# martinResearch/PySparseLP

Hardware: AMD Instinct MI355X
Metric: admm_iterations_per_sec (higher is better)
Workload: dtype f64

## Files before the change

### pysparselp_amd/csrc/slp_tall.h

```cpp
#pragma once
#include "slp_common.h"
#include "slp_tall_item.h"

namespace slp {

constexpr int kTallC = 4096;
constexpr int kTallT = 1024;
constexpr int kTallSlots = 8;
constexpr int kTallDepth = 4;
constexpr int kTallBuckets = 6;
constexpr int kTallCellShift = kTallIdBits + kTallColBits + kTallRowBits;
static_assert(kTallBuckets * 32 == 3 * kWave, "k_tall_build scans the (count, bank class) buckets three per lane of one wave");
static_assert(1 + kTallDictMax + kTallRmax <= (1 << kTallRowBits), "an item's sum field: scratch cell, value table, the block's rows (slp_tall_item.h)");
static_assert(kTallRmax + 1 < (1 << kTallRowBits) && kTallC == (1 << kTallColBits) && kTallDictMax == (1 << kTallIdBits), "tall geometry");
static_assert(kTallT == kTallPlanLanes && kTallC == kTallCmax, "the planner's constants (slp_tall_plan.h)");
static_assert((kTallRmaxSplit + 1) * 8 + kTallDictMax * 8 + 2 * kTallC * 8 <= kTallLdsBytes, "tall cells: LDS budget");

constexpr unsigned int kPktNewCell = 0x80000000u;
constexpr unsigned int kNoTile = 0x7fffffffu;
constexpr unsigned int kOob = 0xffffff00u;

struct TallPkt {
    unsigned int off;
    unsigned int xsrc;
    unsigned int c[4];
    unsigned int strip;
    unsigned int pad;
};
static_assert(sizeof(TallPkt) == 32, "packet header");

__host__ __device__ inline unsigned long long tall_value_key(unsigned long long bits) {
    return (bits >> 63) ? ~bits : (bits | 0x8000000000000000ull);
}

}
```

### pysparselp_amd/csrc/slp_tall.hip

```cpp
#include <atomic>
#include <cmath>
#include <cstdlib>
#include <cstring>
#include <vector>

#include <rocprim/rocprim.hpp>

#include "slp_common.h"
#include "slp_kernels.h"
#include "slp_tall.h"

namespace slp {


__global__ void k_tall_range(i64 nrow, const i64 *__restrict__ ptr, const i32 *__restrict__ idx, i64 c0, i64 c1,
                             i64 *__restrict__ lo, i64 *__restrict__ len) {
    for (i64 r = (i64)blockIdx.x * blockDim.x + threadIdx.x; r < nrow; r += (i64)gridDim.x * blockDim.x) {
        const i64 s = ptr[r], e = ptr[r + 1];
        auto lower = [&](i64 c) {
            i64 a = s, b = e;
            while (a < b) {
                const i64 mid = (a + b) >> 1;
                if ((i64)idx[mid] < c) a = mid + 1;
                else b = mid;
// ... 473 lines not shown
                        tall_scan_put(sc, cell, 2ull, bw + cell_w, bp + cell_p);
                        sc.before_w[cell] = bw;
                        sc.before_p[cell] = bp;
                        s_before_w = bw;
                        s_before_p = bp;
                    }
                }
                __syncthreads();
                SLP_TB_PROF(9);
                if (s_cell < ncell && p * 16 < s_n) {
                    const unsigned int *g = reinterpret_cast<const unsigned int *>(keys + s_c0) + p * 32;
                    const unsigned int lds = __builtin_amdgcn_readfirstlane((unsigned int)(size_t)s_dump);
                    unsigned int m0_saved;
                    asm volatile("s_mov_b32 %0, m0\n\ts_mov_b32 m0, %1\n\ts_nop 0\n\tglobal_load_lds_dword %2, off\n\ts_mov_b32 m0, %0"
                                 : "=&s"(m0_saved) : "s"(lds), "v"(g) : "memory");
                }
                fits = (i64)(s_before_w + cell_w) <= cap_w && (i64)(s_before_p + cell_p) <= cap_p;
                pay = spay + s_before_w;
                payv = DICT ? nullptr : spayv + s_before_w;
                pk = sdir + s_before_p;
            }
            if (!fits) break;
            {
                unsigned int *base = pay + woff;
                unsigned int hb0 = 0, hb1 = 0;
#pragma unroll
                for (int j = 0; j < kTallSlots; ++j) {
                    if ((unsigned)p < wd[REC && j < 4 ? 0 : j]) {
                        unsigned int item = 0u, hib = 0u;
                        if (have >> j & 1u) {
                            const unsigned int r1 = ((unsigned int)(key[j] >> (kTallIdBits + kTallColBits)) & ((1u << kTallRowBits) - 1)) + sum0;
                            const unsigned int cl = (unsigned int)(key[j] >> kTallIdBits) & (kTallC - 1);
                            if (DICT) {
                                const TallItem it = tall_item_encode((unsigned int)key[j] & ((1u << kTallIdBits) - 1), cl, r1);
                                item = it.word;
                                hib = it.fifth;
                            } else {
                                item = tall_item64_encode(cl, r1);
                            }
                        }
                        const unsigned int at = tall_packet_item_word(lay, REC, (unsigned)p, j);
                        base[at] = item;
                        if (!DICT) payv[woff + at] = value[j];
                        if (j < 4) hb0 |= hib << (8 * j);
                        else hb1 |= hib << (8 * (j - 4));
                    }
                }
                if (DICT && (unsigned)p < wd[0]) base[lay.fifth0 + p] = hb0;
                if (DICT && (unsigned)p < wd[4]) base[lay.fifth1 + p] = hb1;
                if (p == 0) {
                    TallPkt h;
                    h.off = woff;
                    h.xsrc = (g == 0) ? (kPktNewCell | tile_of(tn)) : kNoTile;
                    for (int i = 0; i < 4; ++i) h.c[i] = wd[2 * i] | (wd[2 * i + 1] << 16);
                    h.strip = (unsigned int)t;
                    h.pad = 0;
                    pk[npk] = h;
                }
            }
            woff += words;
            ++npk;
            __syncthreads();
            SLP_TB_PROF(10);
        }
    }
}

template <bool DICT>
__global__ __launch_bounds__(kBlock) void k_tall_estimate(i64 ncell, const i64 *__restrict__ cellptr, int records, unsigned long long *__restrict__ est) {
    unsigned long long w = 0, k = 0;
    for (i64 c = (i64)blockIdx.x * kBlock + threadIdx.x; c < ncell; c += (i64)gridDim.x * kBlock) {
        const unsigned long long n = (unsigned long long)(cellptr[c + 1] - cellptr[c]);
        if (!n) continue;
        const unsigned long long L = n < (unsigned)kTallT ? n : (unsigned)kTallT, tau = (n + kTallT - 1) / kTallT;
        const unsigned long long cw = records ? tall_packet_balanced_words(n, kTallT, DICT, true)
                                              : n + L * (tall_packet_lane_words((unsigned int)tau, DICT, false) - tau);
        w += (cw + 3ull) & ~3ull;
        k += (tau + kTallSlots - 1) / kTallSlots;
    }
#pragma unroll
    for (int off = kWave / 2; off; off >>= 1) { w += __shfl_xor(w, off, kWave); k += __shfl_xor(k, off, kWave); }
    if ((threadIdx.x & (kWave - 1)) == 0) { atomicAdd(&est[0], w); atomicAdd(&est[1], k); }
}

__global__ void k_tall_streams(i64 V, i64 T, int S, const i64 *__restrict__ cellptr, TallScan sc, i64 *__restrict__ ext) {
    for (i64 v = (i64)blockIdx.x * blockDim.x + threadIdx.x; v < V; v += (i64)gridDim.x * blockDim.x) {
        const i64 b = v / S, cs = b * T + T * (v % S) / S, ce = b * T + T * (v % S + 1) / S;
        auto before = [&](i64 c, i64 *w, i64 *k) {
            for (--c; c >= 0 && cellptr[c + 1] == cellptr[c];) --c;
            *w = c >= 0 ? (i64)(sc.w[c] & kScanMask) : 0;
            *k = c >= 0 ? (i64)(sc.p[c] & kScanMask) : 0;
        };
        i64 w0, p0, w1, p1;
        before(cs, &w0, &p0);
        before(ce, &w1, &p1);
        ext[4 * v] = w0;
        ext[4 * v + 1] = w1 - w0;
        ext[4 * v + 2] = p0;
        ext[4 * v + 3] = p1 - p0;
    }
}

__global__ void k_tall_dir(i64 ncell, i64 V, i64 T, int S, int C, const i64 *__restrict__ cellptr, TallScan sc, const i64 *__restrict__ ext,
                           const i64 *__restrict__ pkt_ptr, const TallPkt *__restrict__ sdir, TallPkt *__restrict__ dir) {
    const i64 i0 = (i64)blockIdx.x * blockDim.x + threadIdx.x, step = (i64)gridDim.x * blockDim.x;
    for (i64 c = i0; c < ncell; c += step) {
        if (cellptr[c + 1] == cellptr[c]) continue;
        const i64 pk0 = (i64)sc.before_p[c], np = (i64)(sc.p[c] & kScanMask) - pk0, w0 = (i64)sc.before_w[c];
        const i64 b = c / T, t = c % T, v = b * S + (S > 1 ? tall_range_of(t, T, S) : 0);
        TallPkt *out = dir + pkt_ptr[v] + 1 + (pk0 - ext[4 * v + 2]);
        for (i64 j = 0; j < np; ++j) {
            TallPkt h = sdir[pk0 + j];
            h.off += (unsigned int)(w0 - ext[4 * v]);
            out[j] = h;
        }
    }
    for (i64 v = i0; v < V; v += step) {
        const i64 b = v / S, t_begin = T * (v % S) / S, t_end = T * (v % S + 1) / S;
        i64 first = -1;
        for (i64 u = t_begin; u < t_end; ++u)
            if (cellptr[b * T + u + 1] > cellptr[b * T + u]) { first = u; break; }
        TallPkt h;
        h.off = 0; h.xsrc = first >= 0 ? (unsigned int)(first * C) : kNoTile;
        h.c[0] = h.c[1] = h.c[2] = h.c[3] = 0; h.strip = 0; h.pad = 0;
        dir[pkt_ptr[v]] = h;
        h.off = (unsigned int)ext[4 * v + 1];
        h.xsrc = kNoTile;
        for (i64 k = pkt_ptr[v] + 1 + ext[4 * v + 3]; k < pkt_ptr[v + 1]; ++k) dir[k] = h;
    }
}
static int tall_env(const char *name) {
    const char *e = getenv(name);
    return e ? atoi(e) : 0;
}

static i64 tall_pass_nnz() {
    const char *e = getenv("SLP_TALL_PASS_NNZ");
    const i64 v = e ? atoll(e) : 500000000ll;
    return v > 0 ? v : 500000000ll;
}

bool tall_build(const CsrDev &a, bool transposed, StripJds &f, const ValueDict *dict, i64 block_multiple, i64 rows_before, i64 rows_total,
                const TallCarry *carry) {
    Phase ph(transposed ? "tall_build (A^T from the CSR of A)" : "tall_build");
    hipStream_t st = ctx().stream;
    f = StripJds();
    if ((dict && (dict->D <= 0 || dict->D > kTallDictMax)) || a.nrow == 0 || a.ncol == 0 || a.nnz == 0) return false;
    const i64 nrowF = transposed ? a.ncol : a.nrow, ncolF = transposed ? a.nrow : a.ncol;
    if (ncolF * 8 >= ((i64)1 << 31)) return false;
    TallPlanIn pin;
    pin.nrow = nrowF; pin.ncol = ncolF; pin.nnz = a.nnz; pin.D = dict ? dict->D : 0; pin.cus = ctx().num_cu;
    if (!transposed) { pin.block_multiple = block_multiple; pin.rows_before = rows_before; pin.rows_total = rows_total; }
    pin.env_R = std::max(0, tall_env("SLP_TALL_R")); pin.env_C = tall_env("SLP_TALL_C"); pin.env_split = tall_env("SLP_TALL_SPLIT");
    if (const char *e = getenv("SLP_TALL_RECORDS")) pin.env_records = atoi(e) != 0 ? 1 : 0;
    if (carry && carry->C > 0) {
        pin.carry_records = carry->records;
        pin.carry_C = carry->C; pin.carry_dcap = carry->dcap; pin.carry_total = transposed ? 0 : carry->total;
        pin.carry_R = transposed ? carry->R : 0;
        pin.carry_blocks = transposed ? 0 : carry->blocks;
    }
    const TallPlan plan = tall_plan(pin);
    SLP_REQUIRE(plan.lds_bytes <= kTallLdsBytes && plan.build_lds_bytes <= kTallLdsBytes && plan.R >= 1 && plan.R <= kTallRmax,
                "tall_build: the planned geometry does not fit the LDS");
    const int R = plan.R, S = plan.S, Cw = plan.C;
    const bool records = plan.records;
    const i64 T = plan.T;
    const unsigned int sum0 = tall_item_sum_base(plan.dcap);
    SLP_REQUIRE(sum0 + (unsigned int)R <= (1u << kTallRowBits), "tall_build: sum field");
    const i64 B = (nrowF + R - 1) / R, ncell = B * T, V = B * S;
    unsigned int cellbits = 1;
    while (((i64)1 << cellbits) < ncell) ++cellbits;
    if (kTallCellShift + cellbits > 64) return false;
    i64 P = (a.nnz + tall_pass_nnz() - 1) / tall_pass_nnz();
    P = std::max<i64>(1, std::min<i64>(P, B));
    DevBuf<int> bad(1);
    bad.zero();
    if (transposed) {
        hipLaunchKernelGGL(k_tall_sorted, dim3(grid_for(a.nrow * kWave, kBlock)), dim3(kBlock), 0, st, a.nnz, a.idx.p, a.nrow, a.ptr.p, bad.p);
        SLP_HIP(hipGetLastError());
        int hbad = 0;
        bad.download(&hbad, 1);
        if (hbad) return false;
    }
    DevBuf<unsigned long long> sorted((size_t)a.nnz);
    DevBuf<double> svals;
    if (!dict) svals.alloc((size_t)a.nnz);
    {
        Phase p1("  tall: keys + sort");
        DevBuf<i64> lo, len, opos;
        if (transposed) { lo.alloc((size_t)a.nrow); len.alloc((size_t)a.nrow + 1); opos.alloc((size_t)a.nrow + 1); }
        const int D = dict ? dict->D : 0;
        const unsigned long long *dk = dict ? dict->keys.p : (const unsigned long long *)nullptr;
        const unsigned b0 = transposed ? (unsigned)(kTallIdBits + kTallColBits) : (unsigned)kTallCellShift, b1 = (unsigned)kTallCellShift + cellbits;
        i64 done = 0;
        for (i64 pass = 0; pass < P; ++pass) {
            const i64 bb0 = B * pass / P, bb1 = B * (pass + 1) / P;
            if (bb1 == bb0) continue;
            const i64 f0 = bb0 * (i64)R, f1 = std::min<i64>(bb1 * (i64)R, nrowF);
            i64 n_p = 0, obase = 0;
            if (!transposed) {
                i64 ends[2];
                SLP_HIP(hipMemcpyAsync(&ends[0], a.ptr.p + f0, sizeof(i64), hipMemcpyDeviceToHost, st));
                SLP_HIP(hipMemcpyAsync(&ends[1], a.ptr.p + f1, sizeof(i64), hipMemcpyDeviceToHost, st));
                SLP_HIP(hipStreamSynchronize(st));
                obase = ends[0];
                n_p = ends[1] - ends[0];
            } else {
                hipLaunchKernelGGL(k_tall_range, dim3(grid_for(a.nrow, kBlock)), dim3(kBlock), 0, st, a.nrow, a.ptr.p, a.idx.p, f0, f1, lo.p, len.p);
                SLP_HIP(hipGetLastError());
                size_t bytes = 0;
                SLP_HIP(rocprim::exclusive_scan(nullptr, bytes, len.p, opos.p, (i64)0, (size_t)a.nrow + 1, rocprim::plus<i64>(), st));
                DevBuf<char> tmp(bytes);
                SLP_HIP(rocprim::exclusive_scan(tmp.p, bytes, len.p, opos.p, (i64)0, (size_t)a.nrow + 1, rocprim::plus<i64>(), st));
                SLP_HIP(hipMemcpyAsync(&n_p, opos.p + a.nrow, sizeof(i64), hipMemcpyDeviceToHost, st));
                SLP_HIP(hipStreamSynchronize(st));
            }
            if (n_p == 0) continue;
            DevBuf<unsigned long long> keys((size_t)n_p);
            DevBuf<double> kvals;
            if (!dict && transposed) kvals.alloc((size_t)n_p);
            const i64 scan_rows = transposed ? a.nrow : f1 - f0, r0 = transposed ? 0 : f0;
            if (transposed)
                hipLaunchKernelGGL((k_tall_keys<true>), dim3(grid_for(scan_rows * kWave, kBlock)), dim3(kBlock), 0, st, r0, scan_rows, R, T, Cw, (i64)0, D, dk,
                                   a.ptr.p, a.idx.p, a.val.p, lo.p, opos.p, obase, keys.p, kvals.p, bad.p);
            else
                hipLaunchKernelGGL((k_tall_keys<false>), dim3(grid_for(scan_rows * kWave, kBlock)), dim3(kBlock), 0, st, r0, scan_rows, R, T, Cw, (i64)0, D, dk,
                                   a.ptr.p, a.idx.p, a.val.p, (const i64 *)nullptr, (const i64 *)nullptr, obase, keys.p, (double *)nullptr, bad.p);
            SLP_HIP(hipGetLastError());
            size_t bytes = 0;
            if (dict) {
                SLP_HIP(rocprim::radix_sort_keys(nullptr, bytes, keys.p, sorted.p + done, (size_t)n_p, b0, b1, st));
                DevBuf<char> tmp(bytes);
                SLP_HIP(rocprim::radix_sort_keys(tmp.p, bytes, keys.p, sorted.p + done, (size_t)n_p, b0, b1, st));
                SLP_HIP(hipStreamSynchronize(st));
            } else {
                const double *vin = transposed ? kvals.p : a.val.p + obase;
                SLP_HIP(rocprim::radix_sort_pairs(nullptr, bytes, keys.p, sorted.p + done, vin, svals.p + done, (size_t)n_p, b0, b1, st));
                DevBuf<char> tmp(bytes);
                SLP_HIP(rocprim::radix_sort_pairs(tmp.p, bytes, keys.p, sorted.p + done, vin, svals.p + done, (size_t)n_p, b0, b1, st));
                SLP_HIP(hipStreamSynchronize(st));
            }
            done += n_p;
        }
        int hbad = 0;
        bad.download(&hbad, 1);
        if (hbad || done != a.nnz) return false;
    }
    DevBuf<i64> cellptr((size_t)ncell + 1);
    hipLaunchKernelGGL(k_tall_cellptr, dim3(grid_for(a.nnz, kBlock)), dim3(kBlock), 0, st, a.nnz, ncell, sorted.p, cellptr.p);
    SLP_HIP(hipGetLastError());
    Phase p2("  tall: packets (one pass)");
    DevBuf<unsigned long long> scan(4 * (size_t)ncell + 1), est(2);
    TallScan sc;
    sc.w = scan.p; sc.p = scan.p + ncell; sc.ticket = scan.p + 2 * ncell; sc.before_w = sc.ticket + 1; sc.before_p = sc.before_w + ncell;
    est.zero();
    if (dict) hipLaunchKernelGGL((k_tall_estimate<true>), dim3(grid_for(ncell, kBlock)), dim3(kBlock), 0, st, ncell, cellptr.p, records ? 1 : 0, est.p);
    else hipLaunchKernelGGL((k_tall_estimate<false>), dim3(grid_for(ncell, kBlock)), dim3(kBlock), 0, st, ncell, cellptr.p, records ? 1 : 0, est.p);
    SLP_HIP(hipGetLastError());
    unsigned long long hest[2];
    est.download(hest, 2);
    static std::atomic<double> last_needs[2][2][2];
    std::atomic<double> &last_need_slot = last_needs[transposed ? 1 : 0][dict ? 1 : 0][records ? 1 : 0];
    const double last_need = last_need_slot.load();
    const double room = (last_need > 0.5 && last_need < 2.0) ? last_need * 1.003 : 1.10;
    i64 cap_w = (i64)((double)hest[0] * room) + 65536, cap_p = 2 * (i64)hest[1] + 4096;
    if (const char *e = getenv("SLP_TALL_BUILD_ROOM")) cap_w = std::max<i64>(4, (i64)((double)hest[0] * atof(e)));
    i64 tot_w = 0, tot_p = 0;
    DevBuf<i64> ext(4 * (size_t)V);
    std::vector<i64> hext(4 * (size_t)V);
    DevBuf<unsigned int> spay, sdir;
    DevBuf<double> spayv;
    for (int attempt = 0;; ++attempt) {
        spay.release();
        spayv.release();
        spay.alloc((size_t)cap_w + 64);
        sdir.alloc((size_t)cap_p * 8);
        if (!dict) spayv.alloc((size_t)cap_w + 64);
        SLP_HIP(hipMemsetAsync(scan.p, 0, (2 * (size_t)ncell + 1) * sizeof(unsigned long long), st));
        const unsigned grid = (unsigned)std::min<i64>(ncell, (i64)ctx().num_cu);
        auto build = [&](auto kernel) {
            hipLaunchKernelGGL(kernel, dim3(grid), dim3(kTallT), 0, st, R, T, S, Cw, sum0, ncell, sorted.p, dict ? (const double *)nullptr : svals.p, cellptr.p, sc,
                               cap_w, cap_p, reinterpret_cast<TallPkt *>(sdir.p), spay.p, dict ? (double *)nullptr : spayv.p);
        };
        if (dict) { if (records) build(k_tall_build<true, true>); else build(k_tall_build<true, false>); }
        else { if (records) build(k_tall_build<false, true>); else build(k_tall_build<false, false>); }
        hipLaunchKernelGGL(k_tall_streams, dim3(grid_for(V, kBlock)), dim3(kBlock), 0, st, V, T, S, cellptr.p, sc, ext.p);
        SLP_HIP(hipGetLastError());
        ext.download(hext.data(), hext.size());
        tot_w = hext[4 * (V - 1)] + hext[4 * (V - 1) + 1];
        tot_p = hext[4 * (V - 1) + 2] + hext[4 * (V - 1) + 3];
        if (tot_w <= cap_w && tot_p <= cap_p) break;
        SLP_REQUIRE(attempt == 0, "tall_build: the pass with the exact sizes did not fit");
        cap_w = tot_w; cap_p = tot_p;
    }
    sorted.release();
    svals.release();
    std::vector<i64> hbase((size_t)V + 1), hpkt((size_t)V + 1);
    const i64 limit = dict ? ((i64)1 << 28) : ((i64)1 << 27);
    hpkt[0] = 0;
    for (i64 v = 0; v < V; ++v) {
        if (hext[4 * v + 1] >= limit) return false;
        hbase[v] = hext[4 * v];
        const i64 np = 1 + hext[4 * v + 3];
        hpkt[v + 1] = hpkt[v] + (np + 2 * kTallDepth - 1) / (2 * kTallDepth) * (2 * kTallDepth) + 2 * kTallDepth;
    }
    hbase[V] = tot_w;
    DevBuf<i64> dpkt;
    dpkt.upload(hpkt.data(), hpkt.size());
    if (hest[0]) last_need_slot.store((double)tot_w / (double)hest[0]);
    if (cap_w > tot_w + tot_w / 100 + 65536) {
        DevBuf<unsigned int> exact((size_t)tot_w + 64);
        SLP_HIP(hipMemcpyAsync(exact.p, spay.p, (size_t)tot_w * sizeof(unsigned int), hipMemcpyDeviceToDevice, st));
        DevBuf<double> exactv;
        if (!dict) {
            exactv.alloc((size_t)tot_w + 64);
            SLP_HIP(hipMemcpyAsync(exactv.p, spayv.p, (size_t)tot_w * sizeof(double), hipMemcpyDeviceToDevice, st));
        }
        SLP_HIP(hipStreamSynchronize(st));
        spay = std::move(exact);
        spayv = std::move(exactv);
    }
    f.tall_dir.emplace_back((size_t)hpkt[V] * 8);
    f.tall_pay.emplace_back(std::move(spay));
    DevBuf<unsigned int> &dir = f.tall_dir.back(), &pay = f.tall_pay.back();
    double *vals = nullptr;
    if (!dict) { f.tall_val.emplace_back(std::move(spayv)); vals = f.tall_val.back().p; }
    hipLaunchKernelGGL(k_tall_dir, dim3(grid_for(std::max<i64>(ncell, V), kBlock)), dim3(kBlock), 0, st, ncell, V, T, S, Cw, cellptr.p, sc, ext.p, dpkt.p,
                       reinterpret_cast<const TallPkt *>(sdir.p), reinterpret_cast<TallPkt *>(dir.p));
    SLP_HIP(hipGetLastError());
    std::vector<TallWg> wg((size_t)V);
    for (i64 v = 0; v < V; ++v) {
        const i64 b = v / S;
        wg[(size_t)v].dir = dir.p + hpkt[v] * 8;
        wg[(size_t)v].pay = pay.p + hbase[v];
        wg[(size_t)v].val = vals ? vals + hbase[v] : nullptr;
        wg[(size_t)v].dict = nullptr;
        wg[(size_t)v].npk = hpkt[v + 1] - hpkt[v];
        wg[(size_t)v].row0 = (v % S) * nrowF + b * (i64)R;
        wg[(size_t)v].x0 = 0;
        wg[(size_t)v].ncol = ncolF;
        wg[(size_t)v].nrows = (int)std::min<i64>(R, nrowF - b * (i64)R);
        wg[(size_t)v].D = dict ? dict->D : 0;
    }
    if (S > 1 && V > 8) {
        const i64 q = V / 8, r = V % 8;
        std::vector<TallWg> placed((size_t)V);
        for (i64 orig = 0; orig < V; ++orig) {
            const i64 xcd = orig % 8;
            const i64 pos = (xcd < r ? xcd * (q + 1) : r * (q + 1) + (xcd - r) * q) + orig / 8;
            const i64 sr = pos / B, b = pos % B;
            placed[(size_t)orig] = wg[(size_t)(b * S + sr)];
        }
        wg.swap(placed);
    }
    f.tall_wg.upload(wg.data(), wg.size());
    SLP_HIP(hipStreamSynchronize(st));
    f.tall_bytes = (dir.n + (size_t)tot_w) * sizeof(unsigned int) + (vals ? (size_t)tot_w * sizeof(double) : 0) + wg.size() * sizeof(TallWg) +
                   (dict ? (size_t)dict->D * sizeof(double) : 0);
    f.nrow = nrowF; f.ncol = ncolF; f.nnz = a.nnz; f.T = T; f.B = B; f.C = (int)Cw; f.rpl = 1;
    f.D = dict ? dict->D : 0;
    f.dict = dict ? dict->values.p : nullptr;
    f.tall = true;
    f.tall_R = R;
    f.tall_dcap = plan.dcap;
    f.tall_records = records;
    f.tall_total = plan.total;
    f.S = S;
    if (S > 1) f.part.alloc((size_t)S * (size_t)nrowF);
    f.ok = true;
    return true;
}

bool tall_wanted(i64 nrow, i64 ncol, i64 nnz) {
    const char *e = getenv("SLP_TALL");
    if (e && e[0] == '0') return false;
    const char *m = getenv("SLP_STRIP_MIN_NNZ");
    const i64 min_nnz = m ? atoll(m) : 30000000ll;
    if (nnz < min_nnz || nrow <= 0 || ncol <= 0) return false;
    const double per_cell = ((double)nnz / (double)nrow) / (double)((ncol + kTallC - 1) / kTallC);
    return per_cell >= 0.05 && per_cell < 2.5;
}

}
```

### pysparselp_amd/csrc/slp_tall_spmv.hip

```cpp
#include <cmath>
#include <cstdlib>
#include <cstring>
#include <type_traits>
#include <vector>

#include "slp_common.h"
#include "slp_kernels.h"
#include "slp_tall.h"

namespace slp {


template <bool DICT>
struct TallRegs {
    unsigned int lo[kTallSlots];
    unsigned int hi[DICT ? 2 : 1];
    double val[DICT ? 1 : kTallSlots];
    double x[4];
};

template <bool DICT, bool ACC, bool POW = false, int CT = 0, bool REC = false>
__global__ __launch_bounds__(kTallT) void k_tall_spmv(int nseg, const TallWg *__restrict__ wgs, const double *__restrict__ dict_arg,
                                                      const double *__restrict__ x, double *__restrict__ out, double pw, const int cw,
                                                      const int dcap, const int oxt) {
    const int C = CT ? CT : cw;
    constexpr int kDepth = DICT ? kTallDepth : 2;
    extern __shared__ __attribute__((aligned(16))) double tall_lds[];
    double *const dv = tall_lds + kTallItemTableByte / 8;
    double *const acc = tall_lds + tall_item_sum_base(dcap);
    double *const xt = tall_lds + oxt;
    typedef __attribute__((address_space(3))) double lds_double;
    auto lds_at = [](unsigned int a) -> lds_double & { return *(lds_double *)(unsigned long long)a; };
    const unsigned int lds0 = (unsigned int)(unsigned long long)(lds_double *)tall_lds;
    if (lds0 != 0u) __builtin_trap();
    const unsigned int xtb = 8u * (unsigned int)oxt;
    const int p = threadIdx.x;
    const unsigned int wbase = (unsigned int)__builtin_amdgcn_readfirstlane(p & ~(kWave - 1));
    const bool piece0 = (int)wbase < (C >> 1), piece1 = (int)wbase + kTallT < (C >> 1);
    const int v = blockIdx.x;
    int cur = 0;
    TallWg wg = wgs[v];
    if (p == 0) tall_lds[0] = 0.0;
    for (int r = p; r < wg.nrows; r += kTallT) acc[r] = ACC ? out[wg.row0 + r] : 0.0;
  for (int seg = 0; seg < nseg; ++seg) {
    if (seg > 0) wg = wgs[(i64)seg * gridDim.x + v];
    if (DICT) {
        const double *__restrict__ dsrc = dict_arg ? dict_arg : wg.dict;
        for (int q = p; q < wg.D; q += kTallT) dv[q] = dsrc[q];
    }
    typedef const unsigned int __attribute__((address_space(1))) *gptr_t;
    const gptr_t hd = (gptr_t)(unsigned long long)wg.dir + (p & 7);
    const int npk = (int)wg.npk - 2 * kTallDepth;
    const __amdgpu_buffer_rsrc_t rs_x =
        __builtin_amdgcn_make_buffer_rsrc(const_cast<double *>(x + wg.x0), 0, (int)(wg.ncol * 8), 0x00020000);

    typedef unsigned int rsrc_words_t __attribute__((ext_vector_type(4)));
    auto words_of = [](const void *base) {
        const unsigned long long a = (unsigned long long)base;
        rsrc_words_t d;
        d[0] = (unsigned int)a; d[1] = (unsigned int)(a >> 32) & 0xffffu; d[2] = 0u; d[3] = 0x00020000u;
        return d;
    };
    auto as_rsrc = [](const rsrc_words_t &d) {
        __amdgpu_buffer_rsrc_t r;
        __builtin_memcpy(&r, &d, sizeof(r));
        return r;
    };
    rsrc_words_t dpay = words_of(wg.pay), dval = words_of(DICT ? (const void *)x : (const void *)wg.val);
    auto slot_pay = [&](unsigned int end) { dpay[2] = end; return as_rsrc(dpay); };
    auto slot_val = [&](unsigned int end) { dval[2] = 2u * end; return as_rsrc(dval); };

    TallRegs<DICT> regs[kDepth];
    unsigned int hw[kDepth];

    struct TallHdr {
        unsigned int off;
        unsigned int xw;
        unsigned int w[kTallSlots];
    };
    static_assert(kTallT <= (1 << 14), "a width's two bits below its upper half-word are zero: (c >> 14) is 4 x the upper width");
    auto unpack = [&](unsigned int h) {
        TallHdr t;
        t.off = (unsigned int)__builtin_amdgcn_readlane((int)h, 0) * 4u;
        t.xw = (unsigned int)__builtin_amdgcn_readlane((int)h, 1);
#pragma unroll
        for (int i = 0; i < 4; ++i) {
            const unsigned int v = (unsigned int)__builtin_amdgcn_readlane((int)h, 2 + i);
            t.w[2 * i] = (v & 0xffffu) * 4u;
            t.w[2 * i + 1] = v >> 14;
        }
        return t;
    };
    const unsigned int wbytes = wbase * 4u;
    unsigned int xwq[kDepth], c4q[kDepth];

    auto load_tile = [&](TallRegs<DICT> &g, const unsigned int xo) {
#pragma unroll
        for (int i = 0; i < 2; ++i) {
            const unsigned int o = (i == 0 ? piece0 : piece1) && xo != kOob ? xo + (unsigned int)i * (unsigned int)(kTallT * 16) : kOob;
            const auto v = __builtin_amdgcn_raw_buffer_load_b128(rs_x, o, 0, 0);
            g.x[2 * i] = __hiloint2double((int)v[1], (int)v[0]);
            g.x[2 * i + 1] = __hiloint2double((int)v[3], (int)v[2]);
        }
    };

    auto issue_part = [&](TallRegs<DICT> &g, const TallHdr &t, const int part) {
        const unsigned int mine = (unsigned int)p * 4u;
        if (REC && part == 0) {
            const unsigned int so = t.off, end = so + 4u * t.w[0];
            const auto v = __builtin_amdgcn_raw_buffer_load_b128(slot_pay(end), 4u * mine, (int)so, 2);
#pragma unroll
            for (int k = 0; k < 4; ++k) g.lo[k] = v[k];
            if (!DICT) {
#pragma unroll
                for (int h = 0; h < 2; ++h) {
                    const auto u = __builtin_amdgcn_raw_buffer_load_b128(slot_val(end), 8u * mine + 16u * (unsigned int)h, (int)(2u * so), 2);
                    g.val[DICT ? 0 : 2 * h] = __hiloint2double((int)u[1], (int)u[0]);
                    g.val[DICT ? 0 : 2 * h + 1] = __hiloint2double((int)u[3], (int)u[2]);
                }
            }
            if (DICT) g.hi[0] = __builtin_amdgcn_raw_buffer_load_b32(slot_pay(end + t.w[0]), mine, (int)end, 2);
        } else if (part == 0 || wbytes < t.w[4]) {
            unsigned int so = t.off;
            if (part == 1) so += tall_packet_group1_word(t.w, DICT, REC);
#pragma unroll
            for (int k = 4 * part; k < 4 * part + 4; ++k) {
                const unsigned int end = so + t.w[k];
                g.lo[k] = __builtin_amdgcn_raw_buffer_load_b32(slot_pay(end), mine, (int)so, 2);
                if (!DICT) {
                    const auto v = __builtin_amdgcn_raw_buffer_load_b64(slot_val(end), 2u * mine, (int)(2u * so), 2);
                    g.val[DICT ? 0 : k] = __hiloint2double((int)v[1], (int)v[0]);
                }
                so = end;
            }
            if (DICT) {
                if (part == 0) so += t.w[4] + t.w[5] + t.w[6] + t.w[7];
                else if (!REC) so += t.w[0];
                g.hi[DICT ? part : 0] = __builtin_amdgcn_raw_buffer_load_b32(slot_pay(so + t.w[4 * part]), mine, (int)so, 2);
            }
        }
        if (part == 1) {
            const unsigned int xs = t.xw & 0x7fffffffu;
            const unsigned int xo = xs == kNoTile ? kOob : (xs + 2u * (unsigned int)p) * 8u;
            load_tile(g, xo);
        }
    };

    auto consume = [&](TallRegs<DICT> &g, const unsigned int xw, const unsigned int c4, auto &&between) {
        if (xw & kPktNewCell) {
            asm volatile("s_waitcnt lgkmcnt(0)\n\ts_barrier" ::: "memory");
            cur = C - cur;
        }
        auto stage_tile = [&]() {
            if ((xw & 0x7fffffffu) != kNoTile) {
                double *dst = static_cast<double *>(__builtin_assume_aligned(xt + (C - cur) + 2 * p, 16));
                if (piece0) *reinterpret_cast<double2 *>(dst) = make_double2(g.x[0], g.x[1]);
                if (piece1) *reinterpret_cast<double2 *>(dst + 2 * kTallT) = make_double2(g.x[2], g.x[3]);
            }
        };
        stage_tile();
        const unsigned int tileb = xtb + 8u * (unsigned int)cur;
        auto group = [&](const int k0) {
            unsigned int w[4], sa[4];
            double ar[4], pr[4], t[4];
#pragma unroll
            for (int k = 0; k < 4; ++k) {
                w[k] = g.lo[k0 + k];
                sa[k] = (DICT ? tall_item_sum_bytes(w[k], g.hi[DICT ? (k0 >> 2) : 0] >> (8 * k)) : tall_item64_sum_bytes(w[k]));
            }
#pragma unroll
            for (int k = 0; k < 4; ++k) ar[k] = lds_at(sa[k]);
#pragma unroll
            for (int k = 0; k < 4; ++k) {
                unsigned int col = DICT ? tall_item_column(w[k]) : tall_item64_column(w[k]);
                asm("" : "+v"(col));
                const double xv = lds_at((col << 3) + tileb);
                pr[k] = DICT ? lds_at(tall_item_value_bytes(w[k]) + kTallItemTableByte) * xv
                             : (POW ? abs_pow(g.val[DICT ? 0 : k0 + k], pw) * 1.0 : g.val[DICT ? 0 : k0 + k]) * xv;
            }
            t[0] = ar[0] + pr[0];
#pragma unroll
            for (int k = 1; k < 4; ++k) t[k] = ((sa[k] == sa[k - 1]) ? t[k - 1] : ar[k]) + pr[k];
#pragma unroll
            for (int k = 0; k < 4; ++k) lds_at(sa[k]) = t[k];
        };
        group(0);
        between();
        if (wbytes < c4) group(4);
    };

#pragma unroll
    for (int u = 0; u < kDepth; ++u) {
        const TallHdr t = unpack(hd[(i64)u * 8]);
        xwq[u] = t.xw;
        c4q[u] = t.w[4];
        issue_part(regs[u], t, 0);
        issue_part(regs[u], t, 1);
        hw[u] = hd[(i64)(u + kDepth) * 8];
    }
    __syncthreads();
    for (int jj = 0; jj < npk; jj += 2 * kDepth) {
#pragma unroll
        for (int u = 0; u < 2 * kDepth; ++u) {
            const int i = u % kDepth;
            const unsigned int xw = xwq[i], c4 = c4q[i];
            TallHdr t;
            consume(regs[i], xw, c4, [&]() {
                t = unpack(hw[i]);
                xwq[i] = t.xw;
                c4q[i] = t.w[4];
                issue_part(regs[i], t, 0);
            });
            issue_part(regs[i], t, 1);
            hw[i] = hd[(i64)(jj + u + 2 * kDepth) * 8];
        }
    }
    __syncthreads();
  }
    for (int r = p; r < wg.nrows; r += kTallT) out[wg.row0 + r] = acc[r];
}


__global__ void k_tall_combine(i64 nrow, int S, const double *__restrict__ part, double *__restrict__ out, int accum) {
    for (i64 r = (i64)blockIdx.x * blockDim.x + threadIdx.x; r < nrow; r += (i64)gridDim.x * blockDim.x) {
        double a = accum ? out[r] + part[r] : part[r];
        for (int s = 1; s < S; ++s) a += part[(i64)s * nrow + r];
        out[r] = a;
    }
}

template <bool DICT, bool ACC, bool POW>
static void tall_launch(const StripJds &f, unsigned grid, int nseg, const TallWg *wgs, const double *dict, const double *x, double *out, double pw) {
    TallPlan lay;
    lay.R = f.tall_R; lay.C = (int)f.C; lay.dcap = DICT ? f.tall_dcap : 0;
    tall_plan_layout(lay);
    SLP_REQUIRE(tall_width_ok(lay.C) && lay.R > 0 && lay.lds_bytes <= kTallLdsBytes && f.D <= lay.dcap, "tall cells: LDS layout");
    auto go = [&](auto kernel, bool &raised) {
        if (!raised) {
            SLP_HIP(hipFuncSetAttribute(reinterpret_cast<const void *>(kernel), hipFuncAttributeMaxDynamicSharedMemorySize, kTallLdsBytes));
            raised = true;
        }
        hipLaunchKernelGGL(kernel, dim3(grid), dim3(kTallT), (size_t)lay.lds_bytes, ctx().stream, nseg, wgs, dict, x, out, pw, lay.C, lay.dcap,
                           lay.off_xt / 8);
    };
    static bool raised[2][3] = {{false, false, false}, {false, false, false}};
    auto by_width = [&](auto rec) {
        constexpr bool REC = decltype(rec)::value;
        if (DICT && !POW && lay.C == 3072) go(k_tall_spmv<DICT, ACC, POW, (DICT && !POW) ? 3072 : 0, REC>, raised[REC][1]);
        else if (DICT && !POW && lay.C == 4096) go(k_tall_spmv<DICT, ACC, POW, (DICT && !POW) ? 4096 : 0, REC>, raised[REC][2]);
        else go(k_tall_spmv<DICT, ACC, POW, 0, REC>, raised[REC][0]);
    };
    if (f.tall_records) by_width(std::true_type());
    else by_width(std::false_type());
}

void tall_spmv(const StripJds &f, const double *x, double *out, int accum) {
    double *dst = f.S > 1 ? f.part.p : out;
    const unsigned grid = (unsigned)(f.B * f.S);
    const bool acc = accum && f.S == 1;
    const double *none = nullptr;
    if (f.D > 0) { if (acc) tall_launch<true, true, false>(f, grid, 1, f.tall_wg.p, f.dict, x, dst, 0.0); else tall_launch<true, false, false>(f, grid, 1, f.tall_wg.p, f.dict, x, dst, 0.0); }
    else { if (acc) tall_launch<false, true, false>(f, grid, 1, f.tall_wg.p, none, x, dst, 0.0); else tall_launch<false, false, false>(f, grid, 1, f.tall_wg.p, none, x, dst, 0.0); }
    if (f.S > 1)
        hipLaunchKernelGGL(k_tall_combine, dim3(grid_for(f.nrow, kBlock)), dim3(kBlock), 0, ctx().stream, f.nrow, f.S, f.part.p, out, accum);
    SLP_HIP(hipGetLastError());
}

void tall_spmv_fused(const StripJds &f, const double *x, double *out) {
    const int nseg = f.parts_cols ? (int)f.parts.size() : 1;
    const unsigned grid = (unsigned)(f.tall_wg.n / (size_t)nseg);
    if (f.D > 0) tall_launch<true, false, false>(f, grid, nseg, f.tall_wg.p, nullptr, x, out, 0.0);
    else tall_launch<false, false, false>(f, grid, nseg, f.tall_wg.p, nullptr, x, out, 0.0);
    SLP_HIP(hipGetLastError());
}

bool tall_fuse(StripJds &f) {
    f.tall_wg.release();
    const char *e = getenv("SLP_TALL_FUSE");
    if (e && e[0] == '0') return false;
    if (f.parts.empty()) return false;
    const StripJds &f0 = *f.parts[0];
    for (const StripJds *g : f.parts)
        if (!g->ok || !g->tall || g->S != 1 || g->C != f0.C || (g->D > 0) != (f0.D > 0) || g->tall_dcap != f0.tall_dcap ||
            g->tall_records != f0.tall_records ||
            (f.parts_cols && (g->B != f0.B || g->tall_R != f0.tall_R || g->nrow != f0.nrow)))
            return false;
    std::vector<TallWg> all;
    for (size_t k = 0; k < f.parts.size(); ++k) {
        const StripJds &g = *f.parts[k];
        std::vector<TallWg> wg((size_t)g.B);
        SLP_HIP(hipMemcpy(wg.data(), g.tall_wg.p, wg.size() * sizeof(TallWg), hipMemcpyDeviceToHost));
        for (TallWg &w : wg) {
            w.dict = g.dict;
            if (f.parts_cols) w.x0 = f.part_off[k];
            else w.row0 += f.part_off[k];
            all.push_back(w);
        }
    }
    f.tall_wg.upload(all.data(), all.size());
    f.C = f0.C;
    f.tall_dcap = f0.tall_dcap;
    f.tall_records = f0.tall_records;
    f.tall_R = 0;
    for (const StripJds *g : f.parts) f.tall_R = std::max(f.tall_R, g->tall_R);
    return true;
}

void tall_spmv_pow(const StripJds &f, double pw, const double *x, double *out, int accum) {
    SLP_REQUIRE(f.ok && f.tall && f.D == 0, "tall_spmv_pow: not a tall-cell copy with fp64 entries");
    double *dst = f.S > 1 ? f.part.p : out;
    const unsigned grid = (unsigned)(f.B * f.S);
    if (accum && f.S == 1) tall_launch<false, true, true>(f, grid, 1, f.tall_wg.p, nullptr, x, dst, pw);
    else tall_launch<false, false, true>(f, grid, 1, f.tall_wg.p, nullptr, x, dst, pw);
    if (f.S > 1)
        hipLaunchKernelGGL(k_tall_combine, dim3(grid_for(f.nrow, kBlock)), dim3(kBlock), 0, ctx().stream, f.nrow, f.S, f.part.p, out, accum);
    SLP_HIP(hipGetLastError());
}
}
```

Before: 12.08.

## Decouple x-tile prefetch depth and precompute next packet's first item group

Separates the x-tile register buffers from the per-packet payload registers, so tiles are prefetched with their own ring depth (default 2 instead of riding with each of the 4 packets). For the dictionary path, it also computes the next packet's first four items (sum address, column, table value) during the current packet's consume, which hides LDS latency. The host-side packet padding is changed to a multiple of the new loop turn length. This lowers register pressure from tile buffers but adds live registers for the ahead-computed items, and it depends on the next packet's payload having arrived earlier.

```diff
diff --git a/pysparselp_amd/csrc/slp_tall.h b/pysparselp_amd/csrc/slp_tall.h
--- a/pysparselp_amd/csrc/slp_tall.h
+++ b/pysparselp_amd/csrc/slp_tall.h
@@ -7,7 +7,24 @@
 constexpr int kTallC = 4096;
 constexpr int kTallT = 1024;
 constexpr int kTallSlots = 8;
+#if defined(SLP_LAB_VARIANT) && defined(SLP_TALL_DI)
+constexpr int kTallDepth = SLP_TALL_DI;
+#else
 constexpr int kTallDepth = 4;
+#endif
+#if defined(SLP_LAB_VARIANT) && defined(SLP_TALL_DT)
+constexpr int kTallTileDepth = SLP_TALL_DT;
+#else
+constexpr int kTallTileDepth = 2;
+#endif
+#if defined(SLP_LAB_VARIANT) && defined(SLP_TALL_AHEAD)
+constexpr bool kTallAhead = SLP_TALL_AHEAD != 0;
+#else
+constexpr bool kTallAhead = true;
+#endif
+static_assert(kTallTileDepth >= 1 && kTallTileDepth <= kTallDepth, "a tile's source column is taken from the header ring: its packet's header must be unpacked");
+constexpr int tall_lcm(int a, int b) { int m = a; while (m % b) m += a; return m; }
+constexpr int kTallTurn = tall_lcm(2 * kTallDepth, kTallTileDepth);
 constexpr int kTallBuckets = 6;
 constexpr int kTallCellShift = kTallIdBits + kTallColBits + kTallRowBits;
 static_assert(kTallBuckets * 32 == 3 * kWave, "k_tall_build scans the (count, bank class) buckets three per lane of one wave");
diff --git a/pysparselp_amd/csrc/slp_tall.hip b/pysparselp_amd/csrc/slp_tall.hip
--- a/pysparselp_amd/csrc/slp_tall.hip
+++ b/pysparselp_amd/csrc/slp_tall.hip
@@ -799,7 +799,7 @@
         if (hext[4 * v + 1] >= limit) return false;
         hbase[v] = hext[4 * v];
         const i64 np = 1 + hext[4 * v + 3];
-        hpkt[v + 1] = hpkt[v] + (np + 2 * kTallDepth - 1) / (2 * kTallDepth) * (2 * kTallDepth) + 2 * kTallDepth;
+        hpkt[v + 1] = hpkt[v] + (np + kTallTurn - 1) / kTallTurn * kTallTurn + 2 * kTallDepth;
     }
     hbase[V] = tot_w;
     DevBuf<i64> dpkt;
diff --git a/pysparselp_amd/csrc/slp_tall_spmv.hip b/pysparselp_amd/csrc/slp_tall_spmv.hip
--- a/pysparselp_amd/csrc/slp_tall_spmv.hip
+++ b/pysparselp_amd/csrc/slp_tall_spmv.hip
@@ -16,7 +16,13 @@
     unsigned int lo[kTallSlots];
     unsigned int hi[DICT ? 2 : 1];
     double val[DICT ? 1 : kTallSlots];
+};
+struct TallTile {
     double x[4];
+};
+struct TallAheadItems {
+    unsigned int sa[4], col[4];
+    double v[4];
 };
 
 template <bool DICT, bool ACC, bool POW = false, int CT = 0, bool REC = false>
@@ -25,6 +31,10 @@
                                                       const int dcap, const int oxt) {
     const int C = CT ? CT : cw;
     constexpr int kDepth = DICT ? kTallDepth : 2;
+    constexpr int kTileDepth = kTallTileDepth < kDepth ? kTallTileDepth : kDepth;
+    constexpr int kTurn = tall_lcm(2 * kDepth, kTileDepth);
+    constexpr bool AHEAD = DICT && kTallAhead;
+    static_assert(kTallTurn % kTurn == 0, "a workgroup's packets are whole turns of the loop (slp_tall.hip pads to kTallTurn)");
     extern __shared__ __attribute__((aligned(16))) double tall_lds[];
     double *const dv = tall_lds + kTallItemTableByte / 8;
     double *const acc = tall_lds + tall_item_sum_base(dcap);
@@ -71,6 +81,7 @@
     auto slot_val = [&](unsigned int end) { dval[2] = 2u * end; return as_rsrc(dval); };
 
     TallRegs<DICT> regs[kDepth];
+    TallTile tiles[kTileDepth];
     unsigned int hw[kDepth];
 
     struct TallHdr {
@@ -94,7 +105,7 @@
     const unsigned int wbytes = wbase * 4u;
     unsigned int xwq[kDepth], c4q[kDepth];
 
-    auto load_tile = [&](TallRegs<DICT> &g, const unsigned int xo) {
+    auto load_tile = [&](TallTile &g, const unsigned int xo) {
 #pragma unroll
         for (int i = 0; i < 2; ++i) {
             const unsigned int o = (i == 0 ? piece0 : piece1) && xo != kOob ? xo + (unsigned int)i * (unsigned int)(kTallT * 16) : kOob;
@@ -139,14 +150,27 @@
                 g.hi[DICT ? part : 0] = __builtin_amdgcn_raw_buffer_load_b32(slot_pay(so + t.w[4 * part]), mine, (int)so, 2);
             }
         }
-        if (part == 1) {
-            const unsigned int xs = t.xw & 0x7fffffffu;
-            const unsigned int xo = xs == kNoTile ? kOob : (xs + 2u * (unsigned int)p) * 8u;
-            load_tile(g, xo);
-        }
-    };
-
-    auto consume = [&](TallRegs<DICT> &g, const unsigned int xw, const unsigned int c4, auto &&between) {
+    };
+    auto issue_tile = [&](TallTile &g, const unsigned int txw) {
+        const unsigned int xs = txw & 0x7fffffffu;
+        const unsigned int xo = xs == kNoTile ? kOob : (xs + 2u * (unsigned int)p) * 8u;
+        load_tile(g, xo);
+    };
+
+    auto ahead = [&](const TallRegs<DICT> &g, TallAheadItems &d) {
+#pragma unroll
+        for (int k = 0; k < 4; ++k) {
+            const unsigned int w = g.lo[k];
+            d.sa[k] = tall_item_sum_bytes(w, g.hi[0] >> (8 * k));
+            unsigned int col = tall_item_column(w);
+            asm("" : "+v"(col));
+            d.col[k] = col;
+            d.v[k] = lds_at(tall_item_value_bytes(w) + kTallItemTableByte);
+        }
+    };
+
+    auto consume = [&](TallRegs<DICT> &g, const TallRegs<DICT> &gn, TallAheadItems &nx, const TallTile &tile, const unsigned int xw,
+                       const unsigned int c4, auto &&between) {
         if (xw & kPktNewCell) {
             asm volatile("s_waitcnt lgkmcnt(0)\n\ts_barrier" ::: "memory");
             cur = C - cur;
@@ -154,8 +178,8 @@
         auto stage_tile = [&]() {
             if ((xw & 0x7fffffffu) != kNoTile) {
                 double *dst = static_cast<double *>(__builtin_assume_aligned(xt + (C - cur) + 2 * p, 16));
-                if (piece0) *reinterpret_cast<double2 *>(dst) = make_double2(g.x[0], g.x[1]);
-                if (piece1) *reinterpret_cast<double2 *>(dst + 2 * kTallT) = make_double2(g.x[2], g.x[3]);
+                if (piece0) *reinterpret_cast<double2 *>(dst) = make_double2(tile.x[0], tile.x[1]);
+                if (piece1) *reinterpret_cast<double2 *>(dst + 2 * kTallT) = make_double2(tile.x[2], tile.x[3]);
             }
         };
         stage_tile();
@@ -184,7 +208,24 @@
 #pragma unroll
             for (int k = 0; k < 4; ++k) lds_at(sa[k]) = t[k];
         };
-        group(0);
+        auto group_taken = [&]() {
+            double ar[4], pr[4], t[4];
+#pragma unroll
+            for (int k = 0; k < 4; ++k) ar[k] = lds_at(nx.sa[k]);
+#pragma unroll
+            for (int k = 0; k < 4; ++k) pr[k] = nx.v[k] * lds_at((nx.col[k] << 3) + tileb);
+            t[0] = ar[0] + pr[0];
+#pragma unroll
+            for (int k = 1; k < 4; ++k) t[k] = ((nx.sa[k] == nx.sa[k - 1]) ? t[k - 1] : ar[k]) + pr[k];
+#pragma unroll
+            for (int k = 0; k < 4; ++k) lds_at(nx.sa[k]) = t[k];
+        };
+        if (AHEAD) {
+            group_taken();
+            ahead(gn, nx);
+        } else {
+            group(0);
+        }
         between();
         if (wbytes < c4) group(4);
     };
@@ -196,22 +237,26 @@
         c4q[u] = t.w[4];
         issue_part(regs[u], t, 0);
         issue_part(regs[u], t, 1);
+        if (u < kTileDepth) issue_tile(tiles[u], t.xw);
         hw[u] = hd[(i64)(u + kDepth) * 8];
     }
     __syncthreads();
-    for (int jj = 0; jj < npk; jj += 2 * kDepth) {
-#pragma unroll
-        for (int u = 0; u < 2 * kDepth; ++u) {
-            const int i = u % kDepth;
+    TallAheadItems nx;
+    if (AHEAD) ahead(regs[0], nx);
+    for (int jj = 0; jj < npk; jj += kTurn) {
+#pragma unroll
+        for (int u = 0; u < kTurn; ++u) {
+            const int i = u % kDepth, it = u % kTileDepth;
             const unsigned int xw = xwq[i], c4 = c4q[i];
             TallHdr t;
-            consume(regs[i], xw, c4, [&]() {
+            consume(regs[i], regs[(u + 1) % kDepth], nx, tiles[it], xw, c4, [&]() {
                 t = unpack(hw[i]);
                 xwq[i] = t.xw;
                 c4q[i] = t.w[4];
                 issue_part(regs[i], t, 0);
             });
             issue_part(regs[i], t, 1);
+            issue_tile(tiles[it], kTileDepth == kDepth ? t.xw : xwq[(u + kTileDepth) % kDepth]);
             hw[i] = hd[(i64)(jj + u + 2 * kDepth) * 8];
         }
     }
```

Result: faster. 12.25, median of 6 (+1.4%).
